# Orca0917/fine-grained-emotional-control-of-tts

Measured on AMD Instinct MI355X. Metric: train mel-frames/sec at B=32, 80-bin mel; 1/2/4/8 MI355X, higher is better.
Workload: dtype bf16; 1 GPU; FastSpeech2 train step (fwd+loss+bwd+allreduce+AdamW), B=32/GPU, T_phon_max=200, T_mel_max=977, D=384 F=1536 6+6 FFT layers, 80 mels; global_batch=32, seq_len=977, parallelism=dp1

## Files before the change

fine-grained-emotional-control-of-tts_amd/csrc/flash.hip:

```cpp
#include <cstdlib>
#include <type_traits>

#include "fs2_common.h"

typedef __attribute__((ext_vector_type(4))) int i32x4;
__device__ void llvm_raw_buffer_load_lds(i32x4 rsrc, __attribute__((address_space(3))) uint32_t* lds,
                                         int size, int voffset, int soffset, int offset,
                                         int aux) __asm("llvm.amdgcn.raw.buffer.load.lds");

namespace {

typedef __attribute__((ext_vector_type(4))) short s16x4;
typedef __attribute__((ext_vector_type(8))) short s16x8;
typedef __attribute__((address_space(3))) s16x4 lds_s16x4;
constexpr float LOG2E = 1.4426950408889634f;
constexpr int TMAX = 2048;

struct AttnP {
  const bf16* qkv; long ldq;
  const uint8_t* kpad;
  int tiled;
  const bf16* o; long ldo;
  bf16* out; long ldout;
  const bf16* dout; long lddo;
  bf16* dqkv; long lddq;
  float* lse;
  float* dsum;
  int B, H, T, D;
  float scale, scale_log2, p_drop, inv_keep;
  uint32_t seed, salt;
  uint32_t thr16;
  int xflags;
  const int32_t* qbound;
};

__device__ __forceinline__ int attn_qend(const AttnP& p, int b) {
  return p.qbound ? max(0, min(p.T, p.qbound[b])) : p.T;
}

__device__ __forceinline__ bf16x8 ld_frag(const bf16* g) { return *(const bf16x8*)g; }

__device__ __forceinline__ float fexp2(float x) { return __builtin_amdgcn_exp2f(x); }

__device__ __forceinline__ bf16x8 lds_row_frag(const char* t, int rowbytes, int row, int chunk) {
  return *(const bf16x8*)(t + row * rowbytes + ((chunk ^ (row & 7)) << 4));
}

__device__ __forceinline__ bf16x8 lds_tr_frag(const char* t, int rowbytes, int rbase, int m0,
                                              int lane) {
  const int li = lane & 15, g = lane >> 4, q = li >> 2, p = li & 3;
  const int m = m0 + 4 * p;
  const int c = m >> 3, boff = (m & 7) * 2;
  const int k1 = rbase + 4 * g + q, k2 = k1 + 16;
  const char* a1 = t + k1 * rowbytes + ((c ^ (k1 & 7)) << 4) + boff;
  const char* a2 = t + k2 * rowbytes + ((c ^ (k2 & 7)) << 4) + boff;
  const s16x4 lo = __builtin_amdgcn_ds_read_tr16_b64_v4i16((lds_s16x4*)a1);
  const s16x4 hi = __builtin_amdgcn_ds_read_tr16_b64_v4i16((lds_s16x4*)a2);
  const s16x8 v = {lo[0], lo[1], lo[2], lo[3], hi[0], hi[1], hi[2], hi[3]};
  return __builtin_bit_cast(bf16x8, v);
}

__device__ __forceinline__ uint32_t lds_off(const void* p) {
  return (uint32_t)(uintptr_t)(const __attribute__((address_space(3))) char*)p;
}
struct TrFrag { s16x4 lo, hi; };
__device__ __forceinline__ void lds_tr_frag_issue(TrFrag& f, const char* t, int rowbytes, int rbase,
// ... 375 lines not shown
    for (int d = 0; d < 2; ++d)
#pragma unroll
      for (int j = 0; j < 2; ++j) lds_tr_frag_issue(vb[d][j], Vs, DH * 2, 32 * j, 16 * d, lane);
    static_for<0, ND>([&](auto DI) {
      constexpr int d = decltype(DI)::value;
      if constexpr (d + 2 < ND) {
#pragma unroll
        for (int j = 0; j < 2; ++j) lds_tr_frag_issue(vb[(d + 2) % 3][j], Vs, DH * 2, 32 * j, 16 * (d + 2), lane);
        lds_wait<8>(vb[d % 3][0], vb[d % 3][1]);
      } else if constexpr (d + 1 < ND) {
        lds_wait<4>(vb[d % 3][0], vb[d % 3][1]);
      } else {
        lds_wait<0>(vb[d % 3][0], vb[d % 3][1]);
      }
#pragma unroll
      for (int j = 0; j < 2; ++j)
#pragma unroll
        for (int qg = 0; qg < QG; ++qg)
          oacc[d][qg] = __builtin_amdgcn_mfma_f32_16x16x32_bf16(tr_val(vb[d % 3][j]), pf[qg][j], oacc[d][qg], 0, 0, 0);
    });
    __builtin_amdgcn_s_barrier();
  }
#pragma unroll
  for (int qg = 0; qg < QG; ++qg) {
    const float l = xg_sum(lrow[qg]);
    const float inv = p.inv_keep / l;
    const bool qok = qi[qg] < p.T;
    if (qok && g == 0) p.lse[(long)z * p.T + qi[qg]] = mrow[qg] * c + log2f(l);
    bf16* orow = p.out + ((long)b * p.T + (qok ? qi[qg] : 0)) * p.ldout + h * DH;
    store_row_pairs<ND>(orow, oacc, qg, inv, g, qok);
  }
}

template <int DH, int QG, int W8 = 8>
__global__ void __launch_bounds__(W8 * 64 / QG, 1) attn_bwd_dq_kernel(AttnP p) {
  constexpr int NT = W8 * 64 / QG;
  constexpr int NS = DH / 32, ND = DH / 16;
  constexpr int TB = 64 * DH * 2;
  __shared__ __attribute__((aligned(16))) char smem[4 * TB + TMAX + 16];
  uint8_t* kval = (uint8_t*)(smem + 4 * TB);
  int* kbuf = (int*)(smem + 4 * TB + TMAX);
  const int lane = threadIdx.x & 63, wave = threadIdx.x >> 6, g = lane >> 4;
  int blk, z;
  attn_block_coords(blk, z);
  const int b = z / p.H, h = z - b * p.H;
  if (blk * (16 * W8) >= attn_qend(p, b)) {
    for (int i = threadIdx.x; i < 16 * W8 * (DH / 8); i += NT) {
      const int ql = i / (DH / 8), cc = i - ql * (DH / 8);
      const int qr = blk * (16 * W8) + ql;
      if (qr >= p.T) continue;
      *(u32x4*)(p.dqkv + ((long)b * p.T + qr) * p.lddq + h * DH + cc * 8) = u32x4{0u, 0u, 0u, 0u};
    }
    return;
  }
  const uint32_t dkey = fs2_drop_key(p.seed, p.salt);
  const bool drop = p.p_drop > 0.f;
  const bf16* Qb = p.qkv + (long)b * p.T * p.ldq + h * DH;
  const bf16* Kb = Qb + p.D;
  const bf16* Vb = Qb + 2 * p.D;
  const float c = p.scale_log2;

  int qi[QG];
  bf16x8 qf[QG][NS], dof[QG][NS], of[QG][NS];
  float nlse[QG], dsum[QG];
  uint32_t dc[QG][4][2];
#pragma unroll
  for (int qg = 0; qg < QG; ++qg) {
    qi[qg] = blk * (16 * W8) + wave * 16 * QG + qg * 16 + (lane & 15);
    const bool in = qi[qg] < p.T;
    const long ro = (long)b * p.T + (in ? qi[qg] : 0);
#pragma unroll
    for (int s = 0; s < NS; ++s) {
      qf[qg][s] = in ? ld_frag(Qb + (long)qi[qg] * p.ldq + 32 * s + 8 * g) : bf16x8{};
      dof[qg][s] = in ? ld_frag(p.dout + ro * p.lddo + h * DH + 32 * s + 8 * g) : bf16x8{};
      of[qg][s] = in ? ld_frag(p.o + ro * p.ldo + h * DH + 32 * s + 8 * g) : bf16x8{};
    }
    nlse[qg] = in ? -p.lse[(long)z * p.T + qi[qg]] : 0.f;
  }
  TileDma<DH, NT / 64> dma;
  dma.init(wave, lane, p.ldq);
  const i32x4 rsK = make_rsrc(Kb), rsV = make_rsrc(Vb);
  dma.issue(smem, rsK, p.ldq, 0, p.T, wave);
  dma.issue(smem + TB, rsV, p.ldq, 0, p.T, wave);
  int kfull;
  const int kend = build_kvalid(kval, kbuf, p, b, h, &kfull);
#pragma unroll
  for (int qg = 0; qg < QG; ++qg) {
    const bool in = qi[qg] < p.T;
    float dot = 0.f;
#pragma unroll
    for (int s = 0; s < NS; ++s)
#pragma unroll
      for (int e = 0; e < 8; ++e) dot += (float)dof[qg][s][e] * (float)of[qg][s][e];
    dsum[qg] = xg_sum(dot);
    const uint32_t row = (uint32_t)(z * p.T + qi[qg]);
    drop_lane_consts(dc[qg], dkey, row, g);
    if (in && g == 0) {
      p.dsum[(long)z * p.T + qi[qg]] = dsum[qg];
      ((uint32_t*)p.dsum)[(long)p.B * p.H * p.T + (long)z * p.T + qi[qg]] = fs2_attn_rowhash(dkey, row);
    }
  }
  f32x4 qacc[ND][QG];
#pragma unroll
  for (int d = 0; d < ND; ++d)
#pragma unroll
    for (int qg = 0; qg < QG; ++qg) qacc[d][qg] = f32x4{0, 0, 0, 0};
  const int ntile = (kend + 63) / 64;
  asm volatile("s_waitcnt vmcnt(0)" ::: "memory");
  for (int t = 0; t < ntile; ++t) {
    const int k0 = t * 64;
    const char* Ks = smem + (t & 1) * 2 * TB;
    const char* Vs = Ks + TB;
    if (t + 1 < ntile) {
      char* nx = smem + ((t + 1) & 1) * 2 * TB;
      dma.issue(nx, rsK, p.ldq, k0 + 64, p.T, wave);
      dma.issue(nx + TB, rsV, p.ldq, k0 + 64, p.T, wave);
      wait_vmcnt<2 * TileDma<DH, NT / 64>::PER>();
    } else {
      asm volatile("s_waitcnt vmcnt(0)" ::: "memory");
    }
    __builtin_amdgcn_s_barrier();
    __builtin_amdgcn_sched_barrier(0);
    f32x4 sacc[4][QG], pacc[4][QG];
#pragma unroll
    for (int kt = 0; kt < 4; ++kt)
#pragma unroll
      for (int qg = 0; qg < QG; ++qg) { sacc[kt][qg] = f32x4{0, 0, 0, 0}; pacc[kt][qg] = f32x4{0, 0, 0, 0}; }
// ... 123 lines not shown
  for (int s = 0; s < NS; ++s) {
    kf[s] = kin ? ld_frag(Kb + (long)key * p.ldq + 32 * s + 8 * g) : bf16x8{};
    vf[s] = kin ? ld_frag(Vb + (long)key * p.ldq + 32 * s + 8 * g) : bf16x8{};
  }
  f32x4 dk[ND], dv[ND];
#pragma unroll
  for (int d = 0; d < ND; ++d) { dk[d] = f32x4{0, 0, 0, 0}; dv[d] = f32x4{0, 0, 0, 0}; }

  TileDma<DH, W8> dma;
  dma.init(wave, lane, 0);
  const i32x4 rsQ = make_rsrc(Qb), rsO = make_rsrc(dOb);
  const int ntile_all = (attn_qend(p, b) + 63) / 64;
  const long BHT = (long)p.B * p.H * p.T;
  const i32x4 rsL = make_rsrc(p.lse + (long)z * p.T), rsD = make_rsrc(p.dsum + (long)z * p.T);
  const i32x4 rsH = make_rsrc(p.dsum + BHT + (long)z * p.T);
  auto issue_stats = [&](int q0, int buf) {
    if (wave == 0) {
      const int vo = q0 + lane < p.T ? lane * 4 : BUF_OOB;
      blds4(rsL, vo, q0 * 4, (char*)(lsd + buf * 192));
      blds4(rsD, vo, q0 * 4, (char*)(lsd + buf * 192 + 64));
      blds4(rsH, vo, q0 * 4, (char*)(lsd + buf * 192 + 128));
    }
  };
  if (ntile_all > 0) {
    issue_stats(0, 0);
    dma.issue(smem, rsQ, p.ldq, 0, p.T, wave);
    dma.issue(smem + TB, rsO, p.lddo, 0, p.T, wave);
  }
  int kfull;
  build_kvalid(kval, kbuf, p, b, h, &kfull);
  const bool kok = kin && kval[key];
  const int anyk = __syncthreads_or(kok);
  const int ntile = anyk ? ntile_all : 0;
  asm volatile("s_waitcnt vmcnt(0)" ::: "memory");
#ifdef FS2_EXPERIMENTS
  const bool stamps = p.xflags & 64;
  uint64_t st_acc[6] = {0, 0, 0, 0, 0, 0};
  uint64_t st_prev = __builtin_amdgcn_s_memtime();
  const uint64_t st_pro = st_prev - st_entry;
#define FS2_STAMP(i) do { if (stamps) { const uint64_t t_ = __builtin_amdgcn_s_memtime(); st_acc[i] += t_ - st_prev; st_prev = t_; } } while (0)
#else
#define FS2_STAMP(i) do { } while (0)
#endif
  for (int t = 0; t < ntile; ++t) {
    const int q0 = t * 64;
    const char* Qs = smem + (t & 1) * 2 * TB;
    const char* Os = Qs + TB;
    const float* ls_s = lsd + (t & 1) * 192;
    const float* ds_s = ls_s + 64;
    const uint32_t* rh_s = (const uint32_t*)(ls_s + 128);
    if (t + 1 < ntile) {
      issue_stats(q0 + 64, (t + 1) & 1);
      char* nx = smem + ((t + 1) & 1) * 2 * TB;
      dma.issue(nx, rsQ, p.ldq, q0 + 64, p.T, wave);
      dma.issue(nx + TB, rsO, p.lddo, q0 + 64, p.T, wave);
      if (wave == 0) wait_vmcnt<2 * TileDma<DH, W8>::PER + 3>();
      else wait_vmcnt<2 * TileDma<DH, W8>::PER>();
    } else {
      asm volatile("s_waitcnt vmcnt(0)" ::: "memory");
    }
    FS2_STAMP(0);
    __builtin_amdgcn_s_barrier();
    __builtin_amdgcn_sched_barrier(0);
    FS2_STAMP(1);
    f32x4 sacc[4], pacc[4];
#pragma unroll
// ... 13 lines not shown
    for (int qt = 0; qt < 4; ++qt) {
      const f32x4 l4 = *(const f32x4*)(ls_s + qt * 16 + 4 * g);
      const f32x4 d4 = *(const f32x4*)(ds_s + qt * 16 + 4 * g);
      uint32_t hx[4];
      if (drop) {
        const int odd = lane & 1;
        const u32x2 rh2 = *(const u32x2*)(rh_s + qt * 16 + 4 * g + 2 * odd);
        uint32_t mine[2];
#pragma unroll
        for (int e = 0; e < 2; ++e) mine[e] = fs2_attn_mix(rh2[e] + kc);
        uint32_t other[2];
#pragma unroll
        for (int e = 0; e < 2; ++e)
          other[e] = (uint32_t)__builtin_amdgcn_mov_dpp((int)mine[e], 0xB1, 0xF, 0xF, false);
        hx[0] = odd ? other[0] : mine[0];
        hx[1] = odd ? other[1] : mine[1];
        hx[2] = odd ? mine[0] : other[0];
        hx[3] = odd ? mine[1] : other[1];
      }
#pragma unroll
      for (int r = 0; r < 4; ++r) {
        const float pr = fexp2(fmaf(sacc[qt][r], c, -l4[r]));
        float dp = pacc[qt][r];
        float pd = pr;
        if (drop) {
          const bool keep = ((hx[r] >> ((key & 1) * 16)) & 0xffffu) >= p.thr16;
          dp = keep ? dp * p.inv_keep : 0.f;
          pd = keep ? pr : 0.f;
        }
        pdv[qt][r] = pd;
        dsv[qt][r] = pr * (dp - d4[r]);
      }
    }
    bf16x8 pa, sa;
    TrFrag ob[2], qb[2];
    asm volatile("s_waitcnt lgkmcnt(0)" ::: "memory");
    FS2_STAMP(3);
    lds_tr_frag_issue(ob[0], Os, DH * 2, 0, 0, lane);
    lds_tr_frag_issue(qb[0], Qs, DH * 2, 0, 0, lane);
    static_for<0, 2 * ND>([&](auto NI) {
      constexpr int n = decltype(NI)::value, j = n / ND, d = n % ND;
      if constexpr (n + 1 < 2 * ND) {
        constexpr int n1 = n + 1;
        lds_tr_frag_issue(ob[n1 & 1], Os, DH * 2, 32 * (n1 / ND), 16 * (n1 % ND), lane);
        lds_tr_frag_issue(qb[n1 & 1], Qs, DH * 2, 32 * (n1 / ND), 16 * (n1 % ND), lane);
        lds_wait<4>(ob[n & 1], qb[n & 1]);
      } else {
        lds_wait<0>(ob[n & 1], qb[n & 1]);
      }
      if constexpr (d == 0) {
        pa = pack8(pdv[2 * j], pdv[2 * j + 1]);
        sa = pack8(dsv[2 * j], dsv[2 * j + 1]);
      }
      dv[d] = __builtin_amdgcn_mfma_f32_16x16x32_bf16(pa, tr_val(ob[n & 1]), dv[d], 0, 0, 0);
      dk[d] = __builtin_amdgcn_mfma_f32_16x16x32_bf16(sa, tr_val(qb[n & 1]), dk[d], 0, 0, 0);
    });
    FS2_STAMP(4);
    __builtin_amdgcn_s_barrier();
    FS2_STAMP(5);
  }
#ifdef FS2_EXPERIMENTS
  const uint64_t st_loop_end = __builtin_amdgcn_s_memtime();
#endif
  if (ntile > 0) {
    constexpr int RB = 4 * DH;
    static_assert(16 * W8 * RB <= 4 * TB, "dK/dV staging must fit the tile ring");
#pragma unroll
    for (int r = 0; r < 4; ++r) {
      const int kl = wave * 16 + 4 * g + r;
      const bool ok = kval[min(blk * (16 * W8) + kl, p.T - 1)];
      bf16* row = (bf16*)(smem + kl * RB);
#pragma unroll
      for (int d = 0; d < ND; ++d) {
        row[16 * d + (lane & 15)] = (bf16)(ok ? dk[d][r] * p.scale : 0.f);
        row[DH + 16 * d + (lane & 15)] = (bf16)(ok ? dv[d][r] * p.inv_keep : 0.f);
      }
    }
    __syncthreads();
    constexpr int CPR = RB / 16;
    for (int i = threadIdx.x; i < 16 * W8 * CPR; i += W8 * 64) {
      const int kl = i / CPR, cc = i - kl * CPR;
      const int kr = blk * (16 * W8) + kl;
      if (kr >= p.T) continue;
      const int half = cc >= CPR / 2;
      bf16* dst = p.dqkv + ((long)b * p.T + kr) * p.lddq + (1 + half) * p.D + h * DH +
                  (cc - half * (CPR / 2)) * 8;
      *(u32x4*)dst = *(const u32x4*)(smem + kl * RB + cc * 16);
    }
  } else {
    for (int i = threadIdx.x; i < 16 * W8 * (DH / 8) * 2; i += W8 * 64) {
      const int kl = i / (DH / 4), cc = i - kl * (DH / 4);
      const int kr = blk * (16 * W8) + kl;
      if (kr >= p.T) continue;
      const int half = cc >= DH / 8;
      bf16* dst = p.dqkv + ((long)b * p.T + kr) * p.lddq + (1 + half) * p.D + h * DH +
                  (cc - half * (DH / 8)) * 8;
      *(u32x4*)dst = u32x4{0u, 0u, 0u, 0u};
    }
  }
#ifdef FS2_EXPERIMENTS
  if (stamps) {
    asm volatile("s_waitcnt vmcnt(0)" ::: "memory");
    const uint64_t st_end = __builtin_amdgcn_s_memtime();
    if (lane == 0) {
      uint64_t* o = (uint64_t*)(p.dsum + 2L * p.B * p.H * p.T) +
                    ((long)(blockIdx.x + gridDim.x * blockIdx.y) * W8 + wave) * 16;
      for (int i = 0; i < 6; ++i) o[i] = st_acc[i];
      o[6] = ntile;
      o[7] = st_pro;
      o[8] = st_end - st_loop_end;
      o[9] = st_entry;
      o[10] = st_end;
    }
  }
#endif
#undef FS2_STAMP
}

int attn_qg_fwd(int dh) { return dh <= 128 ? 2 : 1; }

bool attn_small_blocks(const AttnP& p) {
  return (long)((p.T + 127) / 128) * p.B * p.H < 256;
}

template <int DH>
void launch_fwd(const AttnP& p, hipStream_t s) {
  if (attn_small_blocks(p)) {
    dim3 grid((p.T + 63) / 64, p.B * p.H);
    if (attn_qg_fwd(DH) == 2) hipLaunchKernelGGL((attn_fwd_kernel<DH, 2, 4>), grid, dim3(128), 0, s, p);
    else hipLaunchKernelGGL((attn_fwd_kernel<DH, 1, 4>), grid, dim3(256), 0, s, p);
    return;
  }
  if constexpr (DH == 192) {
    hipLaunchKernelGGL((attn_fwd_kernel<DH, 2, 16>), dim3((p.T + 255) / 256, p.B * p.H), dim3(512), 0, s, p);
  } else {
    dim3 grid((p.T + 127) / 128, p.B * p.H);
    if (attn_qg_fwd(DH) == 2) hipLaunchKernelGGL((attn_fwd_kernel<DH, 2>), grid, dim3(256), 0, s, p);
    else hipLaunchKernelGGL((attn_fwd_kernel<DH, 1>), grid, dim3(512), 0, s, p);
  }
}
template <int DH>
void launch_bwd(const AttnP& p, hipStream_t s) {
  if (attn_small_blocks(p)) {
    dim3 g1((p.T + 63) / 64, p.B * p.H);
    if constexpr (DH <= 64) hipLaunchKernelGGL((attn_bwd_dq_kernel<DH, 2, 4>), g1, dim3(128), 0, s, p);
    else hipLaunchKernelGGL((attn_bwd_dq_kernel<DH, 1, 4>), g1, dim3(256), 0, s, p);
    hipLaunchKernelGGL((attn_bwd_dkv_kernel<DH, 4>), g1, dim3(256), 0, s, p);
    return;
  }
  dim3 g1((p.T + 127) / 128, p.B * p.H);
  if constexpr (DH <= 64) hipLaunchKernelGGL((attn_bwd_dq_kernel<DH, 2>), g1, dim3(256), 0, s, p);
  else hipLaunchKernelGGL((attn_bwd_dq_kernel<DH, 1>), g1, dim3(512), 0, s, p);
  hipLaunchKernelGGL(attn_bwd_dkv_kernel<DH>, g1, dim3(512), 0, s, p);
}

bool a16(const void* q) { return ((uintptr_t)q & 15) == 0; }

int check(int B, int H, int T, int dh, long ldq, const void* qkv, int dtype) {
  if (dtype != FS2_BF16) return FS2_EINVAL;
  if (B <= 0 || H <= 0 || T <= 0 || T > TMAX) return FS2_EINVAL;
  if (dh != 64 && dh != 128 && dh != 192 && dh != 256) return FS2_EINVAL;
  if (!qkv || !a16(qkv) || (ldq % 8) || ldq < 3L * H * dh) return FS2_EALIGN;
  return 0;
}

}

extern "C" int fs2_attn_supported(int T, int dh, int dtype) {
  return dtype == FS2_BF16 && T > 0 && T <= TMAX &&
         (dh == 64 || dh == 128 || dh == 192 || dh == 256);
}

extern "C" int fs2_attn_fwd(const void* qkv, int64_t ldq, const uint8_t* key_pad, int mask_mode,
                            int B, int H, int T, int dh, float scale, float p_drop, uint32_t seed,
                            uint32_t salt, void* out, int64_t ldo, float* lse, int dtype,
                            void* stream) {
  if (int rc = check(B, H, T, dh, ldq, qkv, dtype)) return rc;
  if (!key_pad || !out || !lse || !a16(out) || (ldo % 8)) return FS2_EINVAL;
  AttnP p{};
  p.qkv = (const bf16*)qkv; p.ldq = ldq; p.kpad = key_pad; p.tiled = mask_mode != 0;
  p.out = (bf16*)out; p.ldout = ldo; p.lse = lse;
  p.B = B; p.H = H; p.T = T; p.D = H * dh;
  p.scale = scale; p.scale_log2 = scale * LOG2E; p.p_drop = p_drop;
  p.inv_keep = p_drop > 0.f ? 1.f / (1.f - p_drop) : 1.f;
  p.seed = seed; p.salt = salt;
  p.thr16 = (uint32_t)(p_drop * 65536.f + 0.5f);
  p.xflags = fs2_exp_int("FS2_ATTN_FLAGS", 0);
  hipStream_t s = (hipStream_t)stream;
  switch (dh) {
    case 64: launch_fwd<64>(p, s); break;
    case 128: launch_fwd<128>(p, s); break;
    case 192: launch_fwd<192>(p, s); break;
    default: launch_fwd<256>(p, s); break;
  }
  FS2_CHECK_LAUNCH();
  return 0;
}

static int attn_bwd_impl(const void* qkv, int64_t ldq, const uint8_t* key_pad, int mask_mode,
                         const void* out, int64_t ldo, const void* dout, int64_t lddo,
                         const float* lse, int B, int H, int T, int dh, float scale,
                         float p_drop, uint32_t seed, uint32_t salt, void* dqkv,
                         int64_t lddq, float* workspace, const int32_t* q_bound, int dtype,
                         void* stream) {
  if (int rc = check(B, H, T, dh, ldq, qkv, dtype)) return rc;
  if (!key_pad || !out || !dout || !lse || !dqkv || !workspace) return FS2_EINVAL;
  if (!a16(out) || !a16(dout) || !a16(dqkv) || (ldo % 8) || (lddo % 8) || (lddq % 8))
    return FS2_EALIGN;
  AttnP p{};
  p.qkv = (const bf16*)qkv; p.ldq = ldq; p.kpad = key_pad; p.tiled = mask_mode != 0;
  p.o = (const bf16*)out; p.ldo = ldo;
  p.dout = (const bf16*)dout; p.lddo = lddo;
  p.dqkv = (bf16*)dqkv; p.lddq = lddq;
  p.lse = (float*)lse; p.dsum = workspace; p.qbound = q_bound;
  p.B = B; p.H = H; p.T = T; p.D = H * dh;
  p.scale = scale; p.scale_log2 = scale * LOG2E; p.p_drop = p_drop;
  p.inv_keep = p_drop > 0.f ? 1.f / (1.f - p_drop) : 1.f;
  p.seed = seed; p.salt = salt;
  p.thr16 = (uint32_t)(p_drop * 65536.f + 0.5f);
  p.xflags = fs2_exp_int("FS2_ATTN_FLAGS", 0);
  hipStream_t s = (hipStream_t)stream;
  switch (dh) {
    case 64: launch_bwd<64>(p, s); break;
    case 128: launch_bwd<128>(p, s); break;
    case 192: launch_bwd<192>(p, s); break;
    default: launch_bwd<256>(p, s); break;
  }
  FS2_CHECK_LAUNCH();
  return 0;
}

extern "C" int fs2_attn_bwd(const void* qkv, int64_t ldq, const uint8_t* key_pad, int mask_mode,
                            const void* out, int64_t ldo, const void* dout, int64_t lddo,
                            const float* lse, int B, int H, int T, int dh, float scale,
                            float p_drop, uint32_t seed, uint32_t salt, void* dqkv,
                            int64_t lddq, float* workspace, int dtype, void* stream) {
  return attn_bwd_impl(qkv, ldq, key_pad, mask_mode, out, ldo, dout, lddo, lse, B, H, T, dh, scale,
                       p_drop, seed, salt, dqkv, lddq, workspace, nullptr, dtype, stream);
}

extern "C" int fs2_attn_bwd_bounded(const void* qkv, int64_t ldq, const uint8_t* key_pad,
                                    int mask_mode, const void* out, int64_t ldo, const void* dout,
                                    int64_t lddo, const float* lse, int B, int H, int T, int dh,
                                    float scale, float p_drop, uint32_t seed, uint32_t salt,
                                    void* dqkv, int64_t lddq, float* workspace,
                                    const int32_t* q_bound, int dtype, void* stream) {
  if (!q_bound) return FS2_EINVAL;
  return attn_bwd_impl(qkv, ldq, key_pad, mask_mode, out, ldo, dout, lddo, lse, B, H, T, dh, scale,
                       p_drop, seed, salt, dqkv, lddq, workspace, q_bound, dtype, stream);
}

extern "C" int64_t fs2_attn_workspace_floats(int B, int H, int T) { return 2 * (int64_t)B * H * T; }

FS2_SEED_SETTER(fs2_seed_base_flash)
```

fine-grained-emotional-control-of-tts_amd/fastspeech2/_native.py:

```python

import ctypes
import os

import torch

_HERE = os.path.dirname(os.path.abspath(__file__))
LIB_PATH = os.environ.get("FS2_HIP_LIB", os.path.join(_HERE, "libfs2_hip.so"))
EXPERIMENTS = os.path.basename(LIB_PATH).startswith("libfs2_hip_exp")


def exp_flag(name, default=False):
    if not EXPERIMENTS:
        return default
    v = os.environ.get(name)
    return default if v is None else v not in ("", "0")


def exp_int(name, default):
    if not EXPERIMENTS:
        return default
    v = os.environ.get(name)
    return default if v is None else int(v)

F32 = 0
# ... 65 lines not shown
        ("tiles_k", ctypes.c_int),
    ]


P = ctypes.c_void_p
I = ctypes.c_int
I64 = ctypes.c_int64
U32 = ctypes.c_uint32
Fl = ctypes.c_float

SIGNATURES = {
    "fs2_gemm": (I, [ctypes.POINTER(GemmDesc), P]),
    "fs2_gemm_plan": (I, [ctypes.POINTER(GemmDesc), ctypes.POINTER(GemmPlanInfo)]),
    "fs2_colsum": (I, [P, I64, I, I, I, P, I, P, P]),
    "fs2_conv_fold": (I, [P, I, I64, I, I, I, I, P, I64, P, I64, P, P, I, P]),
    "fs2_colsum_workspace_floats": (I64, [I, I]),
    "fs2_sum_slices": (I, [P, I, I64, I64, P, I, P]),
    "fs2_pad_transpose": (I, [P, I64, I, I, I, I, I, P, I64, I, P, P, I, P]),
    "fs2_pad_transpose_bounded": (I, [P, I64, I, I, I, I, I, P, I64, I, P, P, P, I, I, P]),
    "fs2_grad_tail_bounds": (I, [P, I, I, I, I, P, P, I, P]),
    "fs2_pad_rows": (I, [P, I64, I, I, I, I, I, I, P, I64, I, P]),
    "fs2_ln_fwd": (I, [P, I64, P, I64, Fl, U32, P, P, P, Fl, I, Fl, U32, P, P, I64, P, I64, P, P,
                       I, I, I, U32, P, I, I, P]),
    "fs2_ln_bwd": (I, [P, I64, P, I64, P, P, P, P, I, Fl, U32, P, I, P, I64, P, Fl, U32, P, P, P,
                       I, I, I, U32, P, P]),
    "fs2_ln_workspace_floats": (I64, [I, I]),
    "fs2_attn_supported": (I, [I, I, I]),
    "fs2_attn_fwd": (I, [P, I64, P, I, I, I, I, I, Fl, Fl, U32, U32, P, I64, P, I, P]),
    "fs2_attn_bwd": (I, [P, I64, P, I, P, I64, P, I64, P, I, I, I, I, Fl, Fl, U32, U32, P, I64,
                         P, I, P]),
    "fs2_attn_bwd_bounded": (I, [P, I64, P, I, P, I64, P, I64, P, I, I, I, I, Fl, Fl, U32, U32, P,
                                 I64, P, P, I, P]),
    "fs2_attn_workspace_floats": (I64, [I, I, I]),
    "fs2_softmax_fwd": (I, [P, P, I, I, I, I, I, I, Fl, Fl, U32, U32, P, P, I, P]),
    "fs2_softmax_bwd": (I, [P, P, I, I, I, I, I, Fl, Fl, U32, U32, P, I, P]),
    "fs2_embed_fwd": (I, [P, P, P, I, I, I, I, P, P, I, P]),
    "fs2_embed_bwd": (I, [P, P, P, I, I, I, P, P, I, P]),
    "fs2_embed_bwd_workspace_floats": (I64, [I, I]),
    "fs2_keypad_from_tokens": (I, [P, I, I, P, P]),
    "fs2_keypad_from_lengths": (I, [P, I, I, P, P, P]),
    "fs2_concat_fwd": (I, [P, P, P, P, I, I, I, I, P, I, I, P]),
    "fs2_concat_bwd_spk": (I, [P, I, P, I, I, I, I, P, I, P, P]),
    "fs2_mask_rows": (I, [P, I64, P, I, I, I, P]),
    "fs2_add3_mask_rows": (I, [P, P, P, I64, P, I, I, I, P]),
    "fs2_rowdot_fwd": (I, [P, I64, P, P, Fl, I, I, P, I, P]),
    "fs2_rowdot_bwd": (I, [P, P, I64, P, Fl, I, I, P, P, P, I, P, P]),
    "fs2_avg_over_durations": (I, [P, I, P, I, I, P, P, P]),
    "fs2_avg_workspace_floats": (I64, [I, I]),
    "fs2_embed1d_fwd": (I, [P, P, P, P, I, I, I, I, P, I, P]),
    "fs2_embed1d_bwd": (I, [P, P, I, I, I, I, P, P, I, P, P]),
    "fs2_lr_index": (I, [P, I, Fl, I, I, I, P, P, P, P]),
    "fs2_lr_gather": (I, [P, P, P, I, I, I, I, P, P, I, P]),
    "fs2_lr_scatter": (I, [P, P, P, I, I, I, I, P, I, P]),
    "fs2_loss_fwd_bwd": (I, [ctypes.POINTER(LossDesc), P]),
    "fs2_loss_workspace_floats": (I64, [I, I, I]),
    "fs2_adamw": (I, [P, P, P, P, I64, Fl, Fl, Fl, Fl, Fl, Fl, Fl, Fl, P]),
    "fs2_weight_prep": (I, [P, I, I, I, I, P, I, P, I, I, P]),
    "fs2_weight_prep_batched": (I, [P, I, I, I, P]),
    "fs2_adamw_prep": (I, [P, I, I, P, I, I, P, P, P, P, Fl, Fl, Fl, Fl, Fl, Fl, Fl, Fl, I, P]),
    "fs2_intensity_input": (I, [P, I, I, I, I, P, I, I, P]),
    "fs2_intensity_head": (I, [P, I64, P, P, P, P, P, I, I, I, I, P, I, P]),
    "fs2_phoneme_average": (I, [P, I, I, P, P, I, I, P, P]),
    "fs2_rank_mixup_input": (I, [P, P, P, I, I, I, P, I, I, P]),
    "fs2_rank_pool": (I, [P, P, P, I, I, I, P, P, P]),
    "fs2_rank_loss_fwd": (I, [P, P, P, P, P, P, P, P, I, I, Fl, Fl, P, P]),
    "fs2_bucket_means": (I, [P, P, P, P, P, I, I, I, P, P]),
# ... 101 lines not shown
```

fine-grained-emotional-control-of-tts_amd/fastspeech2/ops.py:

```python

import collections
import ctypes
import os
import sys

import torch

from . import _native as N

EPC = {N.F32: 4, N.BF16: 8}


def _p(x):
    if x is None:
        return None
    if isinstance(x, int):
        return x
    return x.data_ptr()


def _s():
    return N.stream_ptr()


# ... 176 lines not shown
def ln_ws(M, D):
    return N.lib().fs2_ln_workspace_floats(M, D)


def attn_supported(T, dh, dt):
    return bool(N.lib().fs2_attn_supported(T, dh, dt))


def attn_fwd(qkv, ldq, key_pad, B, H, T, dh, scale, p_drop, seed, salt, out, ldo, lse, *, dt,
             mask_mode=1):
    _chk(N.lib().fs2_attn_fwd(_p(qkv), ldq, _p(key_pad), mask_mode, B, H, T, dh, scale, p_drop,
                              seed & 0xffffffff, salt, _p(out), ldo, _p(lse), dt, _s()),
         "fs2_attn_fwd")


def attn_bwd(qkv, ldq, key_pad, out, ldo, dout, lddo, lse, B, H, T, dh, scale, p_drop, seed, salt,
             dqkv, lddq, *, dt, ws, mask_mode=1, q_bound=None):
    if q_bound is not None:
        assert q_bound.dtype == torch.int32 and q_bound.numel() == B and q_bound.is_contiguous()
        _chk(N.lib().fs2_attn_bwd_bounded(_p(qkv), ldq, _p(key_pad), mask_mode, _p(out), ldo,
                                          _p(dout), lddo, _p(lse), B, H, T, dh, scale, p_drop,
                                          seed & 0xffffffff, salt, _p(dqkv), lddq, _p(ws),
                                          _p(q_bound), dt, _s()), "fs2_attn_bwd_bounded")
        return
    _chk(N.lib().fs2_attn_bwd(_p(qkv), ldq, _p(key_pad), mask_mode, _p(out), ldo, _p(dout), lddo,
                              _p(lse), B, H, T, dh, scale, p_drop, seed & 0xffffffff, salt,
                              _p(dqkv), lddq, _p(ws), dt, _s()), "fs2_attn_bwd")


def attn_ws(B, H, T):
    return N.lib().fs2_attn_workspace_floats(B, H, T)


def softmax_fwd(S, key_pad, B, H, Tq, Tk, ldt, scale, p_drop, seed, salt, P, Pd, *, dt,
                mask_mode=1):
    _chk(N.lib().fs2_softmax_fwd(_p(S), _p(key_pad), mask_mode, B, H, Tq, Tk, ldt, scale, p_drop,
                                 seed & 0xffffffff, salt, _p(P), _p(Pd), dt, _s()), "fs2_softmax_fwd")


def softmax_bwd(dPd, P, B, H, Tq, Tk, ldt, scale, p_drop, seed, salt, dS, *, dt):
    _chk(N.lib().fs2_softmax_bwd(_p(dPd), _p(P), B, H, Tq, Tk, ldt, scale, p_drop,
                                 seed & 0xffffffff, salt, _p(dS), dt, _s()), "fs2_softmax_bwd")


def embed_fwd(tokens, table, pe, pad_idx, B, T, D, X, keep, *, dt):
    _chk(N.lib().fs2_embed_fwd(_p(tokens), _p(table), _p(pe), pad_idx, B, T, D, _p(X), _p(keep),
                               dt, _s()), "fs2_embed_fwd")


def embed_bwd(tokens, dX, keep, M, D, V, dtable, *, dt, ws):
    _chk(N.lib().fs2_embed_bwd(_p(tokens), _p(dX), _p(keep), M, D, V, _p(dtable), _p(ws), dt,
                               _s()), "fs2_embed_bwd")


def embed_bwd_ws(D, V):
    return N.lib().fs2_embed_bwd_workspace_floats(D, V)


def keypad_from_tokens(tokens, pad_idx, M, key_pad):
    _chk(N.lib().fs2_keypad_from_tokens(_p(tokens), pad_idx, M, _p(key_pad), _s()),
         "fs2_keypad_from_tokens")


def keypad_from_lengths(lens, B, T, key_pad, keep=None):
    _chk(N.lib().fs2_keypad_from_lengths(_p(lens), B, T, _p(key_pad), _p(keep), _s()),
         "fs2_keypad_from_lengths")
# ... 230 lines not shown
```

include/fs2_hip.h:

```cpp
#ifndef FS2_HIP_H
#define FS2_HIP_H

#include <stdint.h>

#ifdef __cplusplus
extern "C" {
#endif

#define FS2_F32 0
#define FS2_BF16 1

#define FS2_EINVAL (-1)
#define FS2_EALIGN (-2)

typedef struct fs2_gemm_desc {
  int M, N, K;
  int kvalid;
  int mvalid, nvalid;
  int dtype;
  const void* A; int64_t lda; int a_kmajor;
  const void* B; int64_t ldb; int b_kmajor;
  int conv_mode, conv_t, conv_kw, conv_c;
  void* C; int64_t ldc; int c_fp32;
  int c_conv_kw;
// ... 58 lines not shown
               int64_t ldp, void* y, int64_t ldy, float* mean, float* rstd, int M, int D,
               int dtype, uint32_t seed, void* img, int img_t, int img_p, void* stream);

int fs2_ln_bwd(const void* dy, int64_t lddy, const void* s, int64_t lds, const float* mean,
               const float* rstd, const float* gamma, const float* beta, int do_tanh, float p_o,
               uint32_t salt_o, const float* row_mask, int relu_gate_in, void* ds, int64_t ldds,
               void* dr, float p_r, uint32_t salt_r, float* dgamma, float* dbeta, float* dcol,
               int M, int D,
               int dtype, uint32_t seed, float* workspace, void* stream);
int64_t fs2_ln_workspace_floats(int M, int D);

int fs2_softmax_fwd(const float* S, const uint8_t* key_pad, int mask_mode, int B, int H, int Tq,
                    int Tk, int ldt, float scale, float p_drop, uint32_t seed, uint32_t salt,
                    void* P, void* Pd, int dtype, void* stream);
int fs2_softmax_bwd(const float* dPd, const void* P, int B, int H, int Tq, int Tk, int ldt,
                    float scale, float p_drop, uint32_t seed, uint32_t salt, void* dS, int dtype,
                    void* stream);

int fs2_attn_supported(int T, int dh, int dtype);
int fs2_attn_fwd(const void* qkv, int64_t ldq, const uint8_t* key_pad, int mask_mode, int B,
                 int H, int T, int dh, float scale, float p_drop, uint32_t seed, uint32_t salt,
                 void* out, int64_t ldo, float* lse, int dtype, void* stream);
int fs2_attn_bwd(const void* qkv, int64_t ldq, const uint8_t* key_pad, int mask_mode,
                 const void* out,
                 int64_t ldo, const void* dout, int64_t lddo, const float* lse, int B, int H,
                 int T, int dh, float scale, float p_drop, uint32_t seed, uint32_t salt,
                 void* dqkv, int64_t lddq, float* workspace, int dtype, void* stream);
int fs2_attn_bwd_bounded(const void* qkv, int64_t ldq, const uint8_t* key_pad, int mask_mode,
                         const void* out, int64_t ldo, const void* dout, int64_t lddo,
                         const float* lse, int B, int H, int T, int dh, float scale,
                         float p_drop, uint32_t seed, uint32_t salt, void* dqkv, int64_t lddq,
                         float* workspace, const int32_t* q_bound, int dtype, void* stream);
int64_t fs2_attn_workspace_floats(int B, int H, int T);

int fs2_embed_fwd(const int64_t* tokens, const float* table, const float* pe, int pad_idx,
                  int B, int T, int D, void* X, float* keep, int dtype, void* stream);
int fs2_embed_bwd(const int64_t* tokens, const void* dX, const float* keep, int M, int D,
                  int V, float* dtable, float* workspace, int dtype, void* stream);
int64_t fs2_embed_bwd_workspace_floats(int D, int V);

int fs2_keypad_from_tokens(const int64_t* tokens, int pad_idx, int M, uint8_t* key_pad,
                           void* stream);
int fs2_keypad_from_lengths(const int64_t* lens, int B, int T, uint8_t* key_pad, float* keep,
                            void* stream);

int fs2_concat_fwd(const void* feats, const float* spk_table, const int64_t* spk,
                   const float* intensity, int B, int T, int D, int E, void* cat, int ldc,
                   int dtype, void* stream);
int fs2_concat_bwd_spk(const void* dcat, int ldc, const int64_t* spk, int B, int T, int D,
                       int n_spk, float* dspk, int dtype, float* workspace ,
                       void* stream);

int fs2_mask_rows(void* X, int64_t ldx, const float* keep, int M, int D, int dtype, void* stream);
int fs2_add3_mask_rows(void* X, const void* Y, const void* Z, int64_t ld, const float* keep,
                       int M, int D, int dtype, void* stream);

int fs2_rowdot_fwd(const void* u, int64_t ldu, const float* w, const float* b, float scale, int M,
                   int D, void* y, int dtype, void* stream);
int fs2_rowdot_bwd(const void* dy, const void* u, int64_t ldu, const float* w, float scale, int M,
                   int D, void* du, float* dw, float* db, int dtype, float* workspace,
                   void* stream);

int fs2_avg_over_durations(const float* values, int Tm_in, const int64_t* durs, int B, int Tp,
                           float* avg, float* workspace, void* stream);
int64_t fs2_avg_workspace_floats(int B, int Tm_in);

// ... 118 lines not shown
```

Before: 1.543 million mel-frames/s.

## Materialize dS image in dK/dV kernel and compute dQ from it

Adds a prep kernel that computes the row sums for the backward softmax (and stores kend per head). The dK/dV kernel then writes the dS tile into a bf16 workspace image. A new dQ kernel streams K and the dS image through LDS instead of recomputing QK^T and dO·V^T. This removes the duplicated recomputation in the dQ pass at the cost of writing and reading a B*H*Tp^2 bf16 buffer and a larger workspace. It is gated by an image-size cap.

Measured after the change: 1.555 million mel-frames/s (median of 6 runs). No clear change (+0.8%).

```diff
diff --git a/fine-grained-emotional-control-of-tts_amd/csrc/flash.hip b/fine-grained-emotional-control-of-tts_amd/csrc/flash.hip
--- a/fine-grained-emotional-control-of-tts_amd/csrc/flash.hip
+++ b/fine-grained-emotional-control-of-tts_amd/csrc/flash.hip
@@ -32,6 +32,10 @@
   uint32_t thr16;
   int xflags;
   const int32_t* qbound;
+  bf16* dst;
+  int tp;
+  int* kendws;
+  long ws_floats;
 };
 
 __device__ __forceinline__ int attn_qend(const AttnP& p, int b) {
@@ -473,6 +477,95 @@
   }
 }
 
+template <int NS>
+__device__ __forceinline__ float row_dot(const bf16x8 (&dof)[NS], const bf16x8 (&of)[NS]) {
+  float dot = 0.f;
+#pragma unroll
+  for (int s = 0; s < NS; ++s)
+#pragma unroll
+    for (int e = 0; e < 8; ++e) dot += (float)dof[s][e] * (float)of[s][e];
+  return dot;
+}
+
+template <int DH>
+__global__ void __launch_bounds__(256) attn_bwd_prep_kernel(AttnP p) {
+  constexpr int NS = DH / 32;
+  __shared__ __attribute__((aligned(16))) char smem[TMAX + 16];
+  uint8_t* kval = (uint8_t*)smem;
+  int* kbuf = (int*)(smem + TMAX);
+  const int lane = threadIdx.x & 63, wave = threadIdx.x >> 6, g = lane >> 4;
+  int blk, z;
+  attn_block_coords(blk, z);
+  const int b = z / p.H, h = z - b * p.H;
+  const bool past = blk * 64 >= attn_qend(p, b);
+  const int q = blk * 64 + wave * 16 + (lane & 15);
+  const bool in = q < p.T && !past;
+  const long ro = (long)b * p.T + (in ? q : 0);
+  bf16x8 dof[NS], of[NS];
+#pragma unroll
+  for (int s = 0; s < NS; ++s) {
+    dof[s] = in ? ld_frag(p.dout + ro * p.lddo + h * DH + 32 * s + 8 * g) : bf16x8{};
+    of[s] = in ? ld_frag(p.o + ro * p.ldo + h * DH + 32 * s + 8 * g) : bf16x8{};
+  }
+  int kfull;
+  const int kend = build_kvalid(kval, kbuf, p, b, h, &kfull);
+  if (blk == 0 && threadIdx.x == 0) p.kendws[z] = kend;
+  if (past) return;
+  const uint32_t dkey = fs2_drop_key(p.seed, p.salt);
+  const uint32_t row = (uint32_t)(z * p.T + q);
+  float dsum = xg_sum(row_dot<NS>(dof, of));
+  if (kend > 0 && kend <= 64) {
+    const bool drop = p.p_drop > 0.f;
+    const bf16* Qb = p.qkv + (long)b * p.T * p.ldq + h * DH;
+    const bf16* Kb = Qb + p.D;
+    const bf16* Vb = Qb + 2 * p.D;
+    const float c = p.scale_log2;
+    const float nlse = in ? -p.lse[(long)z * p.T + q] : 0.f;
+    bf16x8 qf[NS];
+#pragma unroll
+    for (int s = 0; s < NS; ++s) qf[s] = in ? ld_frag(Qb + (long)q * p.ldq + 32 * s + 8 * g) : bf16x8{};
+    uint32_t dc[4][2];
+    drop_lane_consts(dc, dkey, row, g);
+    f32x4 sacc[4], pacc[4];
+#pragma unroll
+    for (int kt = 0; kt < 4; ++kt) { sacc[kt] = f32x4{0, 0, 0, 0}; pacc[kt] = f32x4{0, 0, 0, 0}; }
+#pragma unroll
+    for (int s = 0; s < NS; ++s)
+#pragma unroll
+      for (int kt = 0; kt < 4; ++kt) {
+        const int kr = kt * 16 + (lane & 15);
+        const bf16x8 kf = kr < p.T ? ld_frag(Kb + (long)kr * p.ldq + 32 * s + 8 * g) : bf16x8{};
+        const bf16x8 vf = kr < p.T ? ld_frag(Vb + (long)kr * p.ldq + 32 * s + 8 * g) : bf16x8{};
+        sacc[kt] = __builtin_amdgcn_mfma_f32_16x16x32_bf16(kf, qf[s], sacc[kt], 0, 0, 0);
+        pacc[kt] = __builtin_amdgcn_mfma_f32_16x16x32_bf16(vf, dof[s], pacc[kt], 0, 0, 0);
+      }
+    const bool full = 64 <= kfull;
+    float part = 0.f;
+#pragma unroll
+    for (int kt = 0; kt < 4; ++kt) {
+      const uint32_t kw = full ? 0x01010101u : *(const uint32_t*)(kval + kt * 16 + 4 * g);
+#pragma unroll
+      for (int e2 = 0; e2 < 2; ++e2) {
+        const uint32_t hh = drop ? fs2_attn_mix(dc[kt][e2]) : 0u;
+#pragma unroll
+        for (int e = 0; e < 2; ++e) {
+          const int r = 2 * e2 + e;
+          float pr = fexp2(fmaf(sacc[kt][r], c, nlse));
+          if (!full) pr = (kw >> (8 * r)) & 1u ? pr : 0.f;
+          float dp = pacc[kt][r];
+          if (drop) dp = ((hh >> (16 * e)) & 0xffffu) >= p.thr16 ? dp * p.inv_keep : 0.f;
+          part += pr * (dp - dsum);
+        }
+      }
+    }
+    dsum += xg_sum(part);
+  }
+  if (in && g == 0) {
+    p.dsum[(long)z * p.T + q] = dsum;
+    ((uint32_t*)p.dsum)[(long)p.B * p.H * p.T + (long)z * p.T + q] = fs2_attn_rowhash(dkey, row);
+  }
+}
+
 template <int DH, int QG, int W8 = 8>
 __global__ void __launch_bounds__(W8 * 64 / QG, 1) attn_bwd_dq_kernel(AttnP p) {
   constexpr int NT = W8 * 64 / QG;
@@ -528,12 +621,7 @@
 #pragma unroll
   for (int qg = 0; qg < QG; ++qg) {
     const bool in = qi[qg] < p.T;
-    float dot = 0.f;
-#pragma unroll
-    for (int s = 0; s < NS; ++s)
-#pragma unroll
-      for (int e = 0; e < 8; ++e) dot += (float)dof[qg][s][e] * (float)of[qg][s][e];
-    dsum[qg] = xg_sum(dot);
+    dsum[qg] = xg_sum(row_dot<NS>(dof[qg], of[qg]));
     const uint32_t row = (uint32_t)(z * p.T + qi[qg]);
     drop_lane_consts(dc[qg], dkey, row, g);
     if (in && g == 0) {
@@ -723,6 +811,7 @@
   const bool kok = kin && kval[key];
   const int anyk = __syncthreads_or(kok);
   const int ntile = anyk ? ntile_all : 0;
+  bf16* const dsz = p.dst + (long)z * p.tp * p.tp;
   asm volatile("s_waitcnt vmcnt(0)" ::: "memory");
 #ifdef FS2_EXPERIMENTS
   const bool stamps = p.xflags & 64;
@@ -802,6 +891,23 @@
         dsv[qt][r] = pr * (dp - d4[r]);
       }
     }
+    if (p.dst) {
+      int kk = key;
+      asm volatile("" : "+v"(kk));
+      const int dsoff = kk * p.tp + 16 * (g & 1) + 4 * (g - (g & 1)) + q0;
+#pragma unroll
+      for (int j = 0; j < 2; ++j) {
+        const u32x4 sw = __builtin_bit_cast(u32x4, pack8(dsv[2 * j], dsv[2 * j + 1]));
+        u32x2 w[2] = {{kok ? sw[0] : 0u, kok ? sw[1] : 0u}, {kok ? sw[2] : 0u, kok ? sw[3] : 0u}};
+#pragma unroll
+        for (int e = 0; e < 2; ++e) {
+          const auto r = __builtin_amdgcn_permlane16_swap(w[0][e], w[1][e], false, false);
+          w[0][e] = r[0];
+          w[1][e] = r[1];
+        }
+        if (kk < p.tp) *(u32x4*)(dsz + dsoff + 32 * j) = u32x4{w[0][0], w[0][1], w[1][0], w[1][1]};
+      }
+    }
     bf16x8 pa, sa;
     TrFrag ob[2], qb[2];
     asm volatile("s_waitcnt lgkmcnt(0)" ::: "memory");
@@ -858,6 +964,14 @@
       *(u32x4*)dst = *(const u32x4*)(smem + kl * RB + cc * 16);
     }
   } else {
+    if (p.dst && blk * (16 * W8) < kbuf[0]) {
+      const int ncol = ntile_all * 8;
+      for (int i = threadIdx.x; i < 16 * W8 * ncol; i += W8 * 64) {
+        const int kl = i / ncol, cc = i - kl * ncol;
+        const int kr = blk * (16 * W8) + kl;
+        if (kr < p.tp) *(u32x4*)(p.dst + ((long)z * p.tp + kr) * p.tp + cc * 8) = u32x4{0u, 0u, 0u, 0u};
+      }
+    }
     for (int i = threadIdx.x; i < 16 * W8 * (DH / 8) * 2; i += W8 * 64) {
       const int kl = i / (DH / 4), cc = i - kl * (DH / 4);
       const int kr = blk * (16 * W8) + kl;
@@ -873,7 +987,7 @@
     asm volatile("s_waitcnt vmcnt(0)" ::: "memory");
     const uint64_t st_end = __builtin_amdgcn_s_memtime();
     if (lane == 0) {
-      uint64_t* o = (uint64_t*)(p.dsum + 2L * p.B * p.H * p.T) +
+      uint64_t* o = (uint64_t*)(p.dsum + p.ws_floats) +
                     ((long)(blockIdx.x + gridDim.x * blockIdx.y) * W8 + wave) * 16;
       for (int i = 0; i < 6; ++i) o[i] = st_acc[i];
       o[6] = ntile;
@@ -887,6 +1001,124 @@
 #undef FS2_STAMP
 }
 
+template <int NQ, int NW>
+struct DsDma {
+  static constexpr int NI = 64 * NQ * 2 / 1024;
+  static constexpr int PER = NI / NW;
+  static_assert(NI % NW == 0 && NQ >= 64, "image tile instructions must split evenly over the waves");
+  __device__ __forceinline__ static void issue(char* tile, i32x4 rs, int tp, int k0, int ncols,
+                                               int wave, int lane16) {
+#pragma unroll
+    for (int j = 0; j < PER; ++j) {
+      const int o = (wave + j * NW) * 1024 + lane16;
+      const int r = o / (NQ * 2), c = ((o - r * NQ * 2) >> 4) ^ (r & 7);
+      blds16(rs, c * 8 < ncols ? (r * tp + c * 8) * 2 : BUF_OOB, k0 * tp * 2,
+             tile + (wave + j * NW) * 1024);
+    }
+  }
+};
+__device__ __forceinline__ void lds_tie8(TrFrag& a) {
+  asm volatile("s_waitcnt lgkmcnt(8)" : "+v"(a.lo), "+v"(a.hi));
+}
+
+template <int DH, int QG, int NW>
+__global__ void __launch_bounds__(NW * 64, 1) attn_bwd_dq_ds_kernel(AttnP p) {
+  constexpr int NQ = 16 * QG * NW;
+  constexpr int ND = DH / 16;
+  constexpr int TB = 64 * DH * 2, SB = 64 * NQ * 2;
+  static_assert(ND >= 4, "the K^T read ring below runs two blocks ahead");
+  __shared__ __attribute__((aligned(16))) char smem[2 * (TB + SB)];
+  const int lane = threadIdx.x & 63, wave = threadIdx.x >> 6, g = lane >> 4;
+  int blk, z;
+  attn_block_coords(blk, z);
+  const int b = z / p.H, h = z - b * p.H;
+  const int kend = p.kendws[z];
+  const int ntile = (kend + 63) / 64;
+  const int q0 = blk * NQ, qend = attn_qend(p, b);
+  if (q0 >= qend) {
+    for (int i = threadIdx.x; i < NQ * (DH / 8); i += NW * 64) {
+      const int ql = i / (DH / 8), cc = i - ql * (DH / 8);
+      if (q0 + ql >= p.T) continue;
+      *(u32x4*)(p.dqkv + ((long)b * p.T + q0 + ql) * p.lddq + h * DH + cc * 8) = u32x4{0u, 0u, 0u, 0u};
+    }
+    return;
+  }
+  const bf16* Kb = p.qkv + (long)b * p.T * p.ldq + h * DH + p.D;
+  const i32x4 rsK = make_rsrc(Kb);
+  const i32x4 rsS = make_rsrc(p.dst + (long)z * p.tp * p.tp + q0);
+  const int ncols = min(p.tp, (qend + 63) & ~63) - q0;
+  TileDma<DH, NW> dma;
+  dma.init(wave, lane, p.ldq);
+  constexpr int INFL = TileDma<DH, NW>::PER + DsDma<NQ, NW>::PER;
+  dma.issue(smem, rsK, p.ldq, 0, p.T, wave);
+  DsDma<NQ, NW>::issue(smem + TB, rsS, p.tp, 0, ncols, wave, lane * 16);
+  f32x4 qacc[ND][QG];
+#pragma unroll
+  for (int d = 0; d < ND; ++d)
+#pragma unroll
+    for (int qg = 0; qg < QG; ++qg) qacc[d][qg] = f32x4{0, 0, 0, 0};
+  for (int t = 0; t < ntile; ++t) {
+    const char* Ks = smem + (t & 1) * (TB + SB);
+    const char* Ss = Ks + TB;
+    if (t + 1 < ntile) {
+      char* nx = smem + ((t + 1) & 1) * (TB + SB);
+      dma.issue(nx, rsK, p.ldq, 64 * t + 64, p.T, wave);
+      DsDma<NQ, NW>::issue(nx + TB, rsS, p.tp, 64 * t + 64, ncols, wave, lane * 16);
+      wait_vmcnt<INFL>();
+    } else {
+      asm volatile("s_waitcnt vmcnt(0)" ::: "memory");
+    }
+    __builtin_amdgcn_s_barrier();
+    __builtin_amdgcn_sched_barrier(0);
+    TrFrag sb[QG][2], kb2[3][2];
+#pragma unroll
+    for (int qg = 0; qg < QG; ++qg)
+#pragma unroll
+      for (int j = 0; j < 2; ++j)
+        lds_tr_frag_issue(sb[qg][j], Ss, NQ * 2, 32 * j, wave * 16 * QG + 16 * qg, lane);
+#pragma unroll
+    for (int d = 0; d < 2; ++d)
+#pragma unroll
+      for (int j = 0; j < 2; ++j) lds_tr_frag_issue(kb2[d][j], Ks, DH * 2, 32 * j, 16 * d, lane);
+    bf16x8 sf[QG][2];
+    static_for<0, ND>([&](auto DI) {
+      constexpr int d = decltype(DI)::value;
+      if constexpr (d + 2 < ND) {
+#pragma unroll
+        for (int j = 0; j < 2; ++j) lds_tr_frag_issue(kb2[(d + 2) % 3][j], Ks, DH * 2, 32 * j, 16 * (d + 2), lane);
+        lds_wait<8>(kb2[d % 3][0], kb2[d % 3][1]);
+      } else if constexpr (d + 1 < ND) {
+        lds_wait<4>(kb2[d % 3][0], kb2[d % 3][1]);
+      } else {
+        lds_wait<0>(kb2[d % 3][0], kb2[d % 3][1]);
+      }
+      if constexpr (d == 0) {
+#pragma unroll
+        for (int qg = 0; qg < QG; ++qg)
+#pragma unroll
+          for (int j = 0; j < 2; ++j) {
+            lds_tie8(sb[qg][j]);
+            sf[qg][j] = tr_val(sb[qg][j]);
+          }
+      }
+#pragma unroll
+      for (int j = 0; j < 2; ++j)
+#pragma unroll
+        for (int qg = 0; qg < QG; ++qg)
+          qacc[d][qg] = __builtin_amdgcn_mfma_f32_16x16x32_bf16(tr_val(kb2[d % 3][j]), sf[qg][j], qacc[d][qg], 0, 0, 0);
+    });
+    __builtin_amdgcn_s_barrier();
+  }
+  asm volatile("s_waitcnt vmcnt(0)" ::: "memory");
+#pragma unroll
+  for (int qg = 0; qg < QG; ++qg) {
+    const int q = q0 + wave * 16 * QG + qg * 16 + (lane & 15);
+    const bool qok = q < p.T;
+    bf16* row = p.dqkv + ((long)b * p.T + (qok ? q : 0)) * p.lddq + h * DH;
+    store_row_pairs<ND>(row, qacc, qg, p.scale, g, qok);
+  }
+}
+
 int attn_qg_fwd(int dh) { return dh <= 128 ? 2 : 1; }
 
 bool attn_small_blocks(const AttnP& p) {
@@ -910,7 +1142,21 @@
   }
 }
 template <int DH>
+void launch_bwd_ds(const AttnP& p, hipStream_t s) {
+  hipLaunchKernelGGL(attn_bwd_prep_kernel<DH>, dim3((p.T + 63) / 64, p.B * p.H), dim3(256), 0, s, p);
+  if (attn_small_blocks(p)) {
+    dim3 g1((p.T + 63) / 64, p.B * p.H);
+    hipLaunchKernelGGL((attn_bwd_dkv_kernel<DH, 4>), g1, dim3(256), 0, s, p);
+    hipLaunchKernelGGL((attn_bwd_dq_ds_kernel<DH, 2, 2>), g1, dim3(128), 0, s, p);
+    return;
+  }
+  dim3 g1((p.T + 127) / 128, p.B * p.H);
+  hipLaunchKernelGGL(attn_bwd_dkv_kernel<DH>, g1, dim3(512), 0, s, p);
+  hipLaunchKernelGGL((attn_bwd_dq_ds_kernel<DH, 2, 8>), dim3((p.T + 255) / 256, p.B * p.H), dim3(512), 0, s, p);
+}
+template <int DH>
 void launch_bwd(const AttnP& p, hipStream_t s) {
+  if (p.dst) return launch_bwd_ds<DH>(p, s);
   if (attn_small_blocks(p)) {
     dim3 g1((p.T + 63) / 64, p.B * p.H);
     if constexpr (DH <= 64) hipLaunchKernelGGL((attn_bwd_dq_kernel<DH, 2, 4>), g1, dim3(128), 0, s, p);
@@ -925,6 +1171,20 @@
 }
 
 bool a16(const void* q) { return ((uintptr_t)q & 15) == 0; }
+
+constexpr int64_t ATTN_DS_MAX_BYTES = 256LL << 20;
+int64_t attn_ds_image_bytes(int B, int H, int T) {
+  const int64_t tp = (T + 63) / 64 * 64;
+  return (int64_t)B * H * tp * tp * 2;
+}
+bool attn_plan_ds(int B, int H, int T) {
+  if (B <= 0 || H <= 0 || T <= 0 || T > TMAX) return false;
+  if (fs2_exp_int("FS2_ATTN_NO_DS", 0)) return false;
+  return attn_ds_image_bytes(B, H, T) <= ATTN_DS_MAX_BYTES;
+}
+int64_t attn_ws_head(int B, int H, int T) {
+  return (2 * (int64_t)B * H * T + (int64_t)B * H + 3) & ~(int64_t)3;
+}
 
 int check(int B, int H, int T, int dh, long ldq, const void* qkv, int dtype) {
   if (dtype != FS2_BF16) return FS2_EINVAL;
@@ -983,6 +1243,12 @@
   p.dout = (const bf16*)dout; p.lddo = lddo;
   p.dqkv = (bf16*)dqkv; p.lddq = lddq;
   p.lse = (float*)lse; p.dsum = workspace; p.qbound = q_bound;
+  p.tp = (T + 63) / 64 * 64;
+  p.ws_floats = fs2_attn_workspace_floats(B, H, T);
+  if (attn_plan_ds(B, H, T)) {
+    p.kendws = (int*)(workspace + 2 * (int64_t)B * H * T);
+    p.dst = (bf16*)(((uintptr_t)(workspace + attn_ws_head(B, H, T)) + 15) & ~(uintptr_t)15);
+  }
   p.B = B; p.H = H; p.T = T; p.D = H * dh;
   p.scale = scale; p.scale_log2 = scale * LOG2E; p.p_drop = p_drop;
   p.inv_keep = p_drop > 0.f ? 1.f / (1.f - p_drop) : 1.f;
@@ -1020,6 +1286,11 @@
                        p_drop, seed, salt, dqkv, lddq, workspace, q_bound, dtype, stream);
 }
 
-extern "C" int64_t fs2_attn_workspace_floats(int B, int H, int T) { return 2 * (int64_t)B * H * T; }
+extern "C" int fs2_attn_bwd_plan(int B, int H, int T) { return attn_plan_ds(B, H, T) ? 1 : 0; }
+
+extern "C" int64_t fs2_attn_workspace_floats(int B, int H, int T) {
+  if (!attn_plan_ds(B, H, T)) return 2 * (int64_t)B * H * T;
+  return attn_ws_head(B, H, T) + 4 + attn_ds_image_bytes(B, H, T) / 4;
+}
 
 FS2_SEED_SETTER(fs2_seed_base_flash)
diff --git a/fine-grained-emotional-control-of-tts_amd/fastspeech2/_native.py b/fine-grained-emotional-control-of-tts_amd/fastspeech2/_native.py
--- a/fine-grained-emotional-control-of-tts_amd/fastspeech2/_native.py
+++ b/fine-grained-emotional-control-of-tts_amd/fastspeech2/_native.py
@@ -121,6 +121,7 @@
     "fs2_attn_bwd_bounded": (I, [P, I64, P, I, P, I64, P, I64, P, I, I, I, I, Fl, Fl, U32, U32, P,
                                  I64, P, P, I, P]),
     "fs2_attn_workspace_floats": (I64, [I, I, I]),
+    "fs2_attn_bwd_plan": (I, [I, I, I]),
     "fs2_softmax_fwd": (I, [P, P, I, I, I, I, I, I, Fl, Fl, U32, U32, P, P, I, P]),
     "fs2_softmax_bwd": (I, [P, P, I, I, I, I, I, Fl, Fl, U32, U32, P, I, P]),
     "fs2_embed_fwd": (I, [P, P, P, I, I, I, I, P, P, I, P]),
diff --git a/fine-grained-emotional-control-of-tts_amd/fastspeech2/ops.py b/fine-grained-emotional-control-of-tts_amd/fastspeech2/ops.py
--- a/fine-grained-emotional-control-of-tts_amd/fastspeech2/ops.py
+++ b/fine-grained-emotional-control-of-tts_amd/fastspeech2/ops.py
@@ -232,6 +232,10 @@
     return N.lib().fs2_attn_workspace_floats(B, H, T)
 
 
+def attn_bwd_plan(B, H, T):
+    return N.lib().fs2_attn_bwd_plan(B, H, T)
+
+
 def softmax_fwd(S, key_pad, B, H, Tq, Tk, ldt, scale, p_drop, seed, salt, P, Pd, *, dt,
                 mask_mode=1):
     _chk(N.lib().fs2_softmax_fwd(_p(S), _p(key_pad), mask_mode, B, H, Tq, Tk, ldt, scale, p_drop,
diff --git a/include/fs2_hip.h b/include/fs2_hip.h
--- a/include/fs2_hip.h
+++ b/include/fs2_hip.h
@@ -114,6 +114,7 @@
                          float p_drop, uint32_t seed, uint32_t salt, void* dqkv, int64_t lddq,
                          float* workspace, const int32_t* q_bound, int dtype, void* stream);
 int64_t fs2_attn_workspace_floats(int B, int H, int T);
+int fs2_attn_bwd_plan(int B, int H, int T);
 
 int fs2_embed_fwd(const int64_t* tokens, const float* table, const float* pe, int pad_idx,
                   int B, int T, int D, void* X, float* keep, int dtype, void* stream);
```
